# mkshing/e4t-diffusion

Hardware: NVIDIA H100
Metric: E4T pretrain images/sec @512^2 bs16 SD-v1.4 (higher is better)
Workload: dtype bf16

## Files before the change

### e4t-diffusion_b200/csrc/attention.cu

```cuda
#include "attention.cuh"
#include <math.h>
#include <stdlib.h>

static constexpr int kAttnThreads = 128;
static constexpr int kBlk = 64;

template <int DP, int NT = kAttnThreads>
__device__ __forceinline__ void load_rows(bf16* s, const bf16* g, long long ld, int rows_valid, int nrows, int dh) {
  constexpr int CPR = DP / 8, LD = DP + 8;
  const uint32_t sb = smem_u32(s);
  for (int i = threadIdx.x; i < nrows * CPR; i += NT) {
    const int r = i / CPR, c = i - r * CPR;
    const bool ok = r < rows_valid && c * 8 < dh;
    cp_async16(sb + (uint32_t)(r * LD + c * 8) * 2u, ok ? (const void*)(g + (long long)r * ld + c * 8) : (const void*)g,
               ok ? 16u : 0u);
  }
}

__device__ __forceinline__ uint32_t a_addr(const bf16* t, int LD, int row0, int col0) {
  const int l = threadIdx.x & 31;
  return smem_u32(t + (row0 + (l & 15)) * LD + col0 + (l >> 4) * 8);
}
__device__ __forceinline__ uint32_t at_addr(const bf16* t, int LD, int k0, int m0) {
  const int l = threadIdx.x & 31;
// ... 511 lines not shown
    const long long r = i / vpr;
    const int c = (int)(i % vpr) * 8;
    const float4 x = *reinterpret_cast<const float4*>(src + r * C + c);
    const float4 y = *reinterpret_cast<const float4*>(src + r * C + c + 4);
    const long long bb = r / rows_per_b, rr = r % rows_per_b;
    *reinterpret_cast<uint4*>(dst + bb * d_bs + rr * ldd + c) =
        make_uint4(pack_bf16(x.x, x.y), pack_bf16(x.z, x.w), pack_bf16(y.x, y.y), pack_bf16(y.z, y.w));
  }
}

#define E4T_ATTN_DPS(X) X(16) X(32) X(48) X(64) X(80) X(96) X(128) X(160) X(192)
static int attn_dp(int dh) {
  static const int dps[] = {16, 32, 48, 64, 80, 96, 128, 160, 192};
  for (int d : dps)
    if (dh <= d) return d;
  return 0;
}

static int env_int(const char* name, int dflt) {
  const char* e = getenv(name);
  return (e && *e) ? atoi(e) : dflt;
}

static bool attn_use_wgmma(int N, int M, int dh) {
  if (!attn_wgmma_shape_ok(N, M, dh) || !env_int("E4T_ATTN_WGMMA", 1)) return false;
  for (const char* v : {"E4T_ATTN_FWD2", "E4T_ATTN_FWD_PT", "E4T_ATTN_CG", "E4T_ATTN_BWD_FUSED", "E4T_ATTN_BWD_BQ",
                        "E4T_ATTN_BWD_STAGES"})
    if (getenv(v)) return false;
  return true;
}

static int attn_common_checks(int dh, long long ldq, long long ldk, long long ldv) {
  E4T_CHECK(dh % 8 == 0 && dh >= 8 && dh <= 192, "attention: head dim %d unsupported (need dh %% 8 == 0, <= 192)", dh);
  E4T_CHECK(ldq % 8 == 0 && ldk % 8 == 0 && ldv % 8 == 0, "attention: row strides must be multiples of 8 elements");
  return 0;
}

template <typename Kern>
static int attn_launch(Kern kernel, dim3 grid, size_t smem, const AttnArgs& a, cudaStream_t st,
                       int threads = kAttnThreads) {
  E4T_CHECK(smem <= 227 * 1024, "attention: shared memory budget exceeded (%zu)", smem);
  E4T_CUDA(cudaFuncSetAttribute(kernel, cudaFuncAttributeMaxDynamicSharedMemorySize, (int)smem));
  kernel<<<grid, threads, smem, st>>>(a);
  E4T_COUNT_LAUNCH();
  E4T_LAUNCH_CHECK();
  return 0;
}

// ... 7 lines not shown
                                                                     ldo, o_bs, lddo, do_bs);
  E4T_COUNT_LAUNCH();
}

static AttnArgs attn_args(const void* Q, const void* K, const void* V, int B, int H, int N, int M, int dh, long long ldq,
                          long long q_bs, long long ldk, long long k_bs, long long ldv, long long v_bs, float scale) {
  AttnArgs a;
  memset(&a, 0, sizeof(a));
  a.B = B; a.H = H; a.N = N; a.M = M; a.dh = dh; a.scale = scale;
  a.Q = (const bf16*)Q; a.ldq = ldq; a.q_bs = q_bs;
  a.K = (const bf16*)K; a.ldk = ldk; a.k_bs = k_bs;
  a.V = (const bf16*)V; a.ldv = ldv; a.v_bs = v_bs;
  return a;
}

extern "C" int e4t_attn_fwd(const void* Q, const void* K, const void* V, void* O, float* LSE, int B, int H, int N,
                            int M, int dh, long long ldq, long long q_bs, long long ldk, long long k_bs,
                            long long ldv, long long v_bs, long long ldo, long long o_bs, float scale,
                            void* stream_) {
  cudaStream_t st = (cudaStream_t)stream_;
  if (int e = attn_common_checks(dh, ldq, ldk, ldv)) return e;
  AttnArgs a = attn_args(Q, K, V, B, H, N, M, dh, ldq, q_bs, ldk, k_bs, ldv, v_bs, scale);
  a.O = (bf16*)O; a.ldo = ldo; a.o_bs = o_bs; a.LSE = LSE;
  if (attn_use_wgmma(N, M, dh)) return attn_wgmma_fwd(a, st);
  a.stages = 2;
  int warps = 4, cap = 0;
  if (const char* e = getenv("E4T_ATTN_FWD2")) {
    if (e[0] == '0') {
      a.stages = 1;
      warps = 8;
    } else if (e[0] == 'd' || e[0] == 's') {
      a.stages = e[0] == 's' ? 1 : 2;
      a.lazy = 1;
      for (const char* c = e + 1; *c; ++c) {
        if (*c == 'n') a.lazy = 0;
        else if (*c == 'f') warps = 8;
        else if (*c == 'p' && c[1] >= '0' && c[1] <= '8') a.poly = *++c - '0';
      }
    }
  }
  a.p_smem = env_int("E4T_ATTN_FWD_PT", 1) == 0;
  if (const char* e = getenv("E4T_ATTN_CG")) {
    int f = 4, q = 4, k = 4, o = 0;
    sscanf(e, "%d,%d,%d,%d", &f, &q, &k, &o);
    warps = f == 8 ? 8 : 4;
    cap = o > 0 ? o : 0;
  }
// ... 18 lines not shown
static int attn_bwd_impl(const void* Q, const void* K, const void* V, const void* O, const void* dO, const float* LSE,
                         float* Dv, float* dQacc, void* dQ, void* dK, void* dV, int B, int H, int N, int M, int dh,
                         long long ldq, long long q_bs, long long ldk, long long k_bs, long long ldv, long long v_bs,
                         long long ldo, long long o_bs, long long lddo, long long do_bs, long long lddq, long long dq_bs,
                         long long lddk, long long dk_bs, long long lddv, long long dv_bs, float scale, bool fused,
                         bool causal, cudaStream_t st) {
  if (int e = attn_common_checks(dh, ldq, ldk, ldv)) return e;
  E4T_CHECK(lddo % 8 == 0 && lddq % 8 == 0 && lddk % 8 == 0 && lddv % 8 == 0, "e4t_attn_bwd: strides %% 8");
  E4T_CHECK(!causal || N == M, "e4t_attn_bwd_fused_causal: needs N == M");
  AttnArgs a = attn_args(Q, K, V, B, H, N, M, dh, ldq, q_bs, ldk, k_bs, ldv, v_bs, scale);
  a.dO = (const bf16*)dO; a.lddo = lddo; a.do_bs = do_bs;
  a.LSE = const_cast<float*>(LSE); a.Dv = Dv; a.dQacc = dQacc;
  a.dQ = (bf16*)dQ; a.lddq = lddq; a.dq_bs = dq_bs;
  a.dK = (bf16*)dK; a.lddk = lddk; a.dk_bs = dk_bs;
  a.dV = (bf16*)dV; a.lddv = lddv; a.dv_bs = dv_bs;
  launch_attn_delta(O, dO, Dv, B, H, N, dh, ldo, o_bs, lddo, do_bs, st);
  E4T_LAUNCH_CHECK();
  if (fused) E4T_CUDA(cudaMemsetAsync(dQacc, 0, (size_t)B * N * H * dh * sizeof(float), st));
  a.stages = env_int("E4T_ATTN_BWD_STAGES", 2) == 1 ? 1 : 2;
  const bool bq32 = env_int("E4T_ATTN_BWD_BQ", 64) == 32;
  const dim3 gkv(cdiv(M, kBlk), H, B), gq(cdiv(N, kBlk), H, B);
  const int dp = attn_dp(dh);
  int r = -1;
  const bool wg = fused && !causal && attn_use_wgmma(N, M, dh);
  if (wg) r = attn_wgmma_bwd(a, st);
#define E4T_BWD_KV(D, BQ, S)                                                                                     \
  {                                                                                                              \
    const size_t skv = BwdCfg<D, BQ>::smem_bytes(fused);                                                         \
    if (causal) r = attn_launch(attn_bwd_kv_kernel<D, BQ, true, true, S>, gkv, skv, a, st);                      \
    else if (fused) r = attn_launch(attn_bwd_kv_kernel<D, BQ, true, false, S>, gkv, skv, a, st);                 \
    else if (!(r = attn_launch(attn_bwd_kv_kernel<D, BQ, false, false, S>, gkv, skv, a, st)))                    \
      r = attn_launch(attn_bwd_q_kernel<D>, gq, (size_t)6 * kBlk * (D + 8) * 2, a, st);                          \
  }
#define E4T_BWD_BQ(D, BQ)                                                                                        \
  {                                                                                                              \
    if (a.stages == 2) E4T_BWD_KV(D, BQ, 2)                                                                      \
    else E4T_BWD_KV(D, BQ, 1)                                                                                    \
  }
#define E4T_BWD(D)                                                                                               \
  if (!wg && dp == D) {                                                                                               \
    if (D <= 96 && !bq32) E4T_BWD_BQ(D, (D <= 96 ? 64 : 32))                                                      \
    else E4T_BWD_BQ(D, 32)                                                                                       \
  }
  E4T_ATTN_DPS(E4T_BWD)
#undef E4T_BWD
#undef E4T_BWD_BQ
#undef E4T_BWD_KV
// ... 45 lines not shown
```

### e4t-diffusion_b200/csrc/attention.cuh

```cuda
#pragma once
#include "common.cuh"

static constexpr float kLog2e = 1.4426950408889634f;

struct AttnArgs {
  int B, H, N, M, dh;
  float scale;
  int stages, lazy, poly, p_smem;
  const bf16* Q; long long ldq, q_bs;
  const bf16* K; long long ldk, k_bs;
  const bf16* V; long long ldv, v_bs;
  bf16* O; long long ldo, o_bs;
  const bf16* dO; long long lddo, do_bs;
  float* LSE;
  const float* Dv;
  float* dQacc;
  bf16* dQ; long long lddq, dq_bs;
  bf16* dK; long long lddk, dk_bs;
  bf16* dV; long long lddv, dv_bs;
};

bool attn_wgmma_shape_ok(int N, int M, int dh);
int attn_wgmma_fwd(const AttnArgs& a, cudaStream_t st);
int attn_wgmma_bwd(const AttnArgs& a, cudaStream_t st);
```

### e4t-diffusion_b200/csrc/attention_wgmma.cu

```cuda
#include "attention.cuh"
#include "wgmma.cuh"

static constexpr int kWgThreads = 384;
static constexpr int kFwdStages = 3;
static constexpr int kBwdStages = 3;
static constexpr int kTile128 = 128 * 128;
static constexpr int kTile64 = 64 * 128;

__device__ __forceinline__ uint8_t* align1024(uint8_t* p) {
  return p + ((1024u - (smem_u32(p) & 1023u)) & 1023u);
}

__device__ __forceinline__ void fwd_softmax(float (&s)[64], float (&m)[2], float (&l)[2], float (&alpha)[2], float sl2) {
#pragma unroll
  for (int hr = 0; hr < 2; ++hr) {
    float mx = -INFINITY;
#pragma unroll
    for (int j = 0; j < 16; ++j) mx = fmaxf(mx, fmaxf(s[4 * j + 2 * hr], s[4 * j + 2 * hr + 1]));
    mx = fmaxf(mx, __shfl_xor_sync(0xffffffffu, mx, 1));
    mx = fmaxf(mx, __shfl_xor_sync(0xffffffffu, mx, 2));
    const float mnew = fmaxf(m[hr], mx * sl2);
    alpha[hr] = ex2_approx(m[hr] - mnew);
    m[hr] = mnew;
    float rs = 0.f;
#pragma unroll
    for (int j = 0; j < 16; ++j)
#pragma unroll
      for (int e = 0; e < 2; ++e) {
        const float p = ex2_approx(fmaf(s[4 * j + 2 * hr + e], sl2, -mnew));
        s[4 * j + 2 * hr + e] = p;
        rs += p;
      }
    l[hr] = l[hr] * alpha[hr] + rs;
  }
}

template <int NJ>
__device__ __forceinline__ void pack_acc(const float* s, uint32_t* p) {
#pragma unroll
  for (int i = 0; i < 2 * NJ; ++i) p[i] = pack_bf16(s[2 * i], s[2 * i + 1]);
}

template <int DH>
__global__ void __launch_bounds__(kWgThreads, 1)
attn_wgmma_fwd_kernel(const __grid_constant__ CUtensorMap mapQ, const __grid_constant__ CUtensorMap mapK,
                      const __grid_constant__ CUtensorMap mapV, const AttnArgs a) {
  constexpr int KS = (DH + 15) / 16, NO = DH;
  constexpr uint32_t kStage = 2 * kTile128;
  extern __shared__ __align__(1024) uint8_t smem_raw[];
  uint8_t* smem = align1024(smem_raw);
  uint64_t* q_bar = reinterpret_cast<uint64_t*>(smem + kTile128 + kFwdStages * kStage);
  uint64_t* full_bar = q_bar + 1;
  uint64_t* empty_bar = full_bar + kFwdStages;
  const int wg = threadIdx.x >> 7;
  const int b = blockIdx.z, h = blockIdx.y, q0 = blockIdx.x * 128;
  const int nblk = a.M / 128;
  if (threadIdx.x == 0) {
    tma_prefetch_desc(&mapQ);
    tma_prefetch_desc(&mapK);
    tma_prefetch_desc(&mapV);
    mbar_init(q_bar, 1);
    for (int i = 0; i < kFwdStages; ++i) {
      mbar_init(&full_bar[i], 1);
      mbar_init(&empty_bar[i], 256);
    }
    fence_mbar_init();
  }
  __syncthreads();

  if (wg == 0) {
    setmaxnreg_dec<24>();
    if (threadIdx.x != 0) return;
    mbar_expect_tx(q_bar, kTile128);
    tma_load_4d(smem, &mapQ, q_bar, 0, h, q0, b);
    int s = 0;
    uint32_t ph = 0;
    for (int j = 0; j < nblk; ++j) {
      mbar_wait(&empty_bar[s], ph ^ 1u);
      uint8_t* sK = smem + kTile128 + s * kStage;
      mbar_expect_tx(&full_bar[s], kStage);
      tma_load_4d(sK, &mapK, &full_bar[s], 0, h, j * 128, b);
      tma_load_4d(sK + kTile128, &mapV, &full_bar[s], 0, h, j * 128, b);
      if (++s == kFwdStages) {
        s = 0;
        ph ^= 1u;
      }
    }
    return;
  }

  setmaxnreg_inc<240>();
  const int cw = wg - 1;
  const int lane = threadIdx.x & 31, warp = (threadIdx.x >> 5) & 3;
  const uint32_t s0 = smem_u32(smem);
  const uint64_t descQ = wgmma_desc(s0 + kTile64 * cw, 16, 1024);
  const uint64_t descK = wgmma_desc(s0 + kTile128, 16, 1024);
  const uint64_t descV = wgmma_desc(s0 + 2 * kTile128, kTile64, 1024);
  const float sl2 = a.scale * kLog2e;
  float s[64], o[NO / 2];
  uint32_t p[32];
  float m_r[2] = {-INFINITY, -INFINITY}, l_r[2] = {0.f, 0.f}, alpha[2];
#pragma unroll
  for (int i = 0; i < NO / 2; ++i) o[i] = 0.f;

  auto issue_qk = [&](int st) {
    const uint64_t dk = descK + (uint64_t)(st * (kStage >> 4));
#pragma unroll
    for (int k = 0; k < KS; ++k) Wgmma<128, 0, 0>::mma(s, descQ + (uint64_t)(2 * k), dk + (uint64_t)(2 * k), k > 0);
    wgmma_commit();
  };

  mbar_wait(q_bar, 0);
  mbar_wait(&full_bar[0], 0);
  wgmma_fence();
  issue_qk(0);
  wgmma_wait<0>();
  reg_fence<64>(s);
  fwd_softmax(s, m_r, l_r, alpha, sl2);
  pack_acc<16>(s, p);

  auto issue_pv = [&](int st) {
    const uint64_t dv = descV + (uint64_t)(st * (kStage >> 4));
#pragma unroll
    for (int kk = 0; kk < 8; ++kk) WgmmaRS<NO, 1>::mma(o, p + 4 * kk, dv + (uint64_t)(kk * (2048 >> 4)), 1);
    wgmma_commit();
  };
  int st = 0;
  uint32_t ph = 0;
  for (int j = 0; j + 1 < nblk; ++j) {
    int sn = st + 1;
    uint32_t phn = ph;
// ... 35 lines not shown
  reg_fence_u32<32>(p);

#pragma unroll
  for (int hr = 0; hr < 2; ++hr) {
    float l = l_r[hr];
    l += __shfl_xor_sync(0xffffffffu, l, 1);
    l += __shfl_xor_sync(0xffffffffu, l, 2);
    const int row = q0 + 64 * cw + 16 * warp + (lane >> 2) + 8 * hr;
    const float inv = 1.f / l;
    bf16* orow = a.O + b * a.o_bs + (long long)row * a.ldo + h * DH;
#pragma unroll
    for (int dt = 0; dt < DH / 8; ++dt)
      *reinterpret_cast<uint32_t*>(orow + dt * 8 + 2 * (lane & 3)) =
          pack_bf16(o[4 * dt + 2 * hr] * inv, o[4 * dt + 2 * hr + 1] * inv);
    if ((lane & 3) == 0) a.LSE[((long long)b * a.H + h) * a.N + row] = (m_r[hr] + log2f(l)) * (1.f / kLog2e);
  }
}

template <int DH>
__global__ void __launch_bounds__(kWgThreads, 1)
attn_wgmma_bwd_kernel(const __grid_constant__ CUtensorMap mapQ, const __grid_constant__ CUtensorMap mapK,
                      const __grid_constant__ CUtensorMap mapV, const __grid_constant__ CUtensorMap mapdO,
                      const __grid_constant__ CUtensorMap mapdQ, const AttnArgs a) {
  constexpr int KS = (DH + 15) / 16, NO = DH, BQ = 64;
  constexpr uint32_t kStage = 2 * kTile64;
  constexpr uint32_t kOffQ = 2 * kTile128;
  constexpr uint32_t kOffdS = kOffQ + kBwdStages * kStage;
  constexpr uint32_t kOffdQ = kOffdS + 2 * kTile128;
  constexpr uint32_t kdQBytes = BQ * DH * 4;
  constexpr uint32_t kOffL = kOffdQ + 2 * kdQBytes;
  constexpr uint32_t kOffBar = kOffL + kBwdStages * 2 * BQ * 4;
  static_assert(kOffdQ % 128 == 0 && kdQBytes % 128 == 0 && kOffL % 16 == 0 && kOffBar % 8 == 0, "smem layout");
  extern __shared__ __align__(1024) uint8_t smem_raw[];
  uint8_t* smem = align1024(smem_raw);
  float* sL = reinterpret_cast<float*>(smem + kOffL);
  uint64_t* kv_bar = reinterpret_cast<uint64_t*>(smem + kOffBar);
  uint64_t* full_bar = kv_bar + 1;
  uint64_t* empty_bar = full_bar + kBwdStages;
  uint64_t* ds_full = empty_bar + kBwdStages;
  uint64_t* ds_empty = ds_full + 2;
  const int wg = threadIdx.x >> 7;
  const int b = blockIdx.z, h = blockIdx.y, k0 = blockIdx.x * 128;
  const int lane = threadIdx.x & 31, warp = (threadIdx.x >> 5) & 3;
  const int nq = a.N / BQ;
  const long long bh = (long long)b * a.H + h;
  if (threadIdx.x == 0) {
    tma_prefetch_desc(&mapQ);
    tma_prefetch_desc(&mapK);
    tma_prefetch_desc(&mapV);
    tma_prefetch_desc(&mapdO);
    tma_prefetch_desc(&mapdQ);
    mbar_init(kv_bar, 1);
    for (int i = 0; i < kBwdStages; ++i) {
      mbar_init(&full_bar[i], 1);
      mbar_init(&empty_bar[i], 256);
    }
    for (int i = 0; i < 2; ++i) {
      mbar_init(&ds_full[i], 256);
      mbar_init(&ds_empty[i], 128);
    }
    fence_mbar_init();
  }
  __syncthreads();
  const uint32_t s0 = smem_u32(smem);

  if (wg == 0) {
    setmaxnreg_dec<72>();
    auto load_block = [&](int i) {
      const int s = i % kBwdStages;
      mbar_wait(&empty_bar[s], ((uint32_t)(i / kBwdStages) & 1u) ^ 1u);
      uint8_t* sQ = smem + kOffQ + s * kStage;
      mbar_expect_tx(&full_bar[s], kStage + 2 * BQ * 4);
      tma_load_4d(sQ, &mapQ, &full_bar[s], 0, h, i * BQ, b);
      tma_load_4d(sQ + kTile64, &mapdO, &full_bar[s], 0, h, i * BQ, b);
      bulk_load_1d(sL + s * 2 * BQ, a.LSE + bh * a.N + i * BQ, BQ * 4, &full_bar[s]);
      bulk_load_1d(sL + s * 2 * BQ + BQ, a.Dv + bh * a.N + i * BQ, BQ * 4, &full_bar[s]);
    };
    if (threadIdx.x == 0) {
      mbar_expect_tx(kv_bar, 2 * kTile128);
      tma_load_4d(smem, &mapK, kv_bar, 0, h, k0, b);
      tma_load_4d(smem + kTile128, &mapV, kv_bar, 0, h, k0, b);
      for (int i = 0; i < kBwdStages - 1 && i < nq; ++i) load_block(i);
    }
    __syncwarp();
    const uint64_t descS = wgmma_desc(s0 + kOffdS, kTile64, 1024);
    const uint64_t descK = wgmma_desc(s0, kTile64, 1024);
    mbar_wait(kv_bar, 0);
    float dq[NO / 2];
    for (int i = 0; i < nq; ++i) {
      const int buf = i & 1;
      if (threadIdx.x == 0 && i + kBwdStages - 1 < nq) load_block(i + kBwdStages - 1);
      __syncwarp();
      mbar_wait(&ds_full[buf], (uint32_t)(i >> 1) & 1u);
      const uint64_t da = descS + (uint64_t)(buf * (kTile128 >> 4));
      wgmma_fence();
#pragma unroll
      for (int kk = 0; kk < 8; ++kk)
        Wgmma<NO, 1, 1>::mma(dq, da + (uint64_t)(kk * (2048 >> 4)), descK + (uint64_t)(kk * (2048 >> 4)), kk > 0);
      wgmma_commit();
      wgmma_wait<0>();
      reg_fence<NO / 2>(dq);
      mbar_arrive(&ds_empty[buf]);
      if (threadIdx.x == 0) tma_store_wait_read<1>();
      named_bar_sync(1, 128);
      float* stg = reinterpret_cast<float*>(smem + kOffdQ + buf * kdQBytes);
#pragma unroll
      for (int hr = 0; hr < 2; ++hr) {
        float* row = stg + (16 * warp + (lane >> 2) + 8 * hr) * DH + 2 * (lane & 3);
#pragma unroll
        for (int dt = 0; dt < DH / 8; ++dt)
          *reinterpret_cast<float2*>(row + 8 * dt) =
              make_float2(dq[4 * dt + 2 * hr] * a.scale, dq[4 * dt + 2 * hr + 1] * a.scale);
      }
      fence_proxy_async_smem();
      named_bar_sync(1, 128);
      if (threadIdx.x == 0) {
        tma_reduce_add_3d(&mapdQ, stg, h * DH, i * BQ, b);
        tma_store_commit();
      }
    }
    if (threadIdx.x == 0) tma_store_wait_all();
    return;
  }

  setmaxnreg_inc<216>();
  const int cw = wg - 1;
  const uint64_t descKa = wgmma_desc(s0 + kTile64 * cw, 16, 1024);
  const uint64_t descVa = wgmma_desc(s0 + kTile128 + kTile64 * cw, 16, 1024);
  const uint64_t descQk = wgmma_desc(s0 + kOffQ, 16, 1024);
  const uint64_t descQm = wgmma_desc(s0 + kOffQ, kTile64, 1024);
  const float sl2 = a.scale * kLog2e;
  float st[32], dpt[32], dk[NO / 2], dv[NO / 2];
  uint32_t pp[16], ps[16];
#pragma unroll
  for (int i = 0; i < NO / 2; ++i) dk[i] = dv[i] = 0.f;
  const int r0 = 64 * cw + 16 * warp + (lane >> 2);
  mbar_wait(kv_bar, 0);
  for (int i = 0; i < nq; ++i) {
    const int s = i % kBwdStages, buf = i & 1;
    mbar_wait(&full_bar[s], (uint32_t)(i / kBwdStages) & 1u);
    const uint64_t so = (uint64_t)(s * (kStage >> 4));
    reg_fence<32>(st);
    reg_fence<32>(dpt);
    wgmma_fence();
#pragma unroll
    for (int k = 0; k < KS; ++k)
      Wgmma<64, 0, 0>::mma(st, descKa + (uint64_t)(2 * k), descQk + so + (uint64_t)(2 * k), k > 0);
    wgmma_commit();
#pragma unroll
    for (int k = 0; k < KS; ++k)
      Wgmma<64, 0, 0>::mma(dpt, descVa + (uint64_t)(2 * k), descQk + so + (uint64_t)((kTile64 >> 4) + 2 * k), k > 0);
    wgmma_commit();
    const float* l_s = sL + s * 2 * BQ + 2 * (lane & 3);
    wgmma_wait<1>();
    reg_fence<32>(st);
#pragma unroll
    for (int j = 0; j < 8; ++j) {
      const float2 l = *reinterpret_cast<const float2*>(l_s + 8 * j);
      const float l0 = l.x * kLog2e, l1 = l.y * kLog2e;
      st[4 * j] = ex2_approx(fmaf(st[4 * j], sl2, -l0));
      st[4 * j + 1] = ex2_approx(fmaf(st[4 * j + 1], sl2, -l1));
      st[4 * j + 2] = ex2_approx(fmaf(st[4 * j + 2], sl2, -l0));
      st[4 * j + 3] = ex2_approx(fmaf(st[4 * j + 3], sl2, -l1));
    }
    pack_acc<8>(st, pp);
    wgmma_wait<0>();
    reg_fence<32>(dpt);
#pragma unroll
    for (int j = 0; j < 8; ++j) {
      const float2 d = *reinterpret_cast<const float2*>(l_s + BQ + 8 * j);
      dpt[4 * j] = st[4 * j] * (dpt[4 * j] - d.x);
      dpt[4 * j + 1] = st[4 * j + 1] * (dpt[4 * j + 1] - d.y);
      dpt[4 * j + 2] = st[4 * j + 2] * (dpt[4 * j + 2] - d.x);
      dpt[4 * j + 3] = st[4 * j + 3] * (dpt[4 * j + 3] - d.y);
    }
    pack_acc<8>(dpt, ps);
    mbar_wait(&ds_empty[buf], ((uint32_t)(i >> 1) & 1u) ^ 1u);
    uint8_t* sdS = smem + kOffdS + buf * kTile128;
#pragma unroll
    for (int j = 0; j < 8; ++j) {
      *reinterpret_cast<uint32_t*>(sdS + sw128_off(r0, j) + 4 * (lane & 3)) = ps[2 * j];
      *reinterpret_cast<uint32_t*>(sdS + sw128_off(r0 + 8, j) + 4 * (lane & 3)) = ps[2 * j + 1];
    }
    fence_proxy_async_smem();
    mbar_arrive(&ds_full[buf]);
    reg_fence<NO / 2>(dk);
    reg_fence<NO / 2>(dv);
    wgmma_fence();
#pragma unroll
    for (int kq = 0; kq < 4; ++kq)
      WgmmaRS<NO, 1>::mma(dv, pp + 4 * kq, descQm + so + (uint64_t)((kTile64 >> 4) + kq * (2048 >> 4)), 1);
#pragma unroll
    for (int kq = 0; kq < 4; ++kq) WgmmaRS<NO, 1>::mma(dk, ps + 4 * kq, descQm + so + (uint64_t)(kq * (2048 >> 4)), 1);
    wgmma_commit();
    wgmma_wait<0>();
    reg_fence<NO / 2>(dk);
    reg_fence<NO / 2>(dv);
    reg_fence_u32<16>(pp);
    reg_fence_u32<16>(ps);
    mbar_arrive(&empty_bar[s]);
  }
#pragma unroll
  for (int hr = 0; hr < 2; ++hr) {
    const int key = k0 + r0 + 8 * hr;
    bf16* dkr = a.dK + b * a.dk_bs + (long long)key * a.lddk + h * DH + 2 * (lane & 3);
    bf16* dvr = a.dV + b * a.dv_bs + (long long)key * a.lddv + h * DH + 2 * (lane & 3);
#pragma unroll
    for (int dt = 0; dt < DH / 8; ++dt) {
      *reinterpret_cast<uint32_t*>(dkr + 8 * dt) = pack_bf16(dk[4 * dt + 2 * hr] * a.scale, dk[4 * dt + 2 * hr + 1] * a.scale);
      *reinterpret_cast<uint32_t*>(dvr + 8 * dt) = pack_bf16(dv[4 * dt + 2 * hr], dv[4 * dt + 2 * hr + 1]);
    }
  }
}

bool attn_wgmma_shape_ok(int N, int M, int dh) {
  return dh == 40 && N >= 512 && M >= 512 && N % 128 == 0 && M % 128 == 0;
}

static int head_map(CUtensorMap* m, const bf16* p, const AttnArgs& a, int tokens, long long ld, long long bs, int rows) {
  E4T_CHECK(((uintptr_t)p & 15) == 0 && ld % 8 == 0 && bs % 8 == 0,
            "attention (wgmma): tensors must be 16-byte aligned with strides that are multiples of 8 elements");
  const uint64_t dims[4] = {(uint64_t)a.dh, (uint64_t)a.H, (uint64_t)tokens, (uint64_t)a.B};
  const uint64_t str[3] = {(uint64_t)a.dh * 2, (uint64_t)ld * 2, (uint64_t)bs * 2};
  const uint32_t box[4] = {64, 1, (uint32_t)rows, 1};
  return e4t_tmap_encode(m, p, 4, dims, str, box, 2);
}

int attn_wgmma_fwd(const AttnArgs& a, cudaStream_t st) {
  CUtensorMap mQ, mK, mV;
  if (int e = head_map(&mQ, a.Q, a, a.N, a.ldq, a.q_bs, 128)) return e;
  if (int e = head_map(&mK, a.K, a, a.M, a.ldk, a.k_bs, 128)) return e;
  if (int e = head_map(&mV, a.V, a, a.M, a.ldv, a.v_bs, 128)) return e;
  E4T_CHECK(a.ldo % 2 == 0 && a.o_bs % 2 == 0, "attention (wgmma): output strides must be even");
  const size_t smem = 1024 + kTile128 + kFwdStages * 2 * kTile128 + 64;
  auto kernel = attn_wgmma_fwd_kernel<40>;
  E4T_CUDA(cudaFuncSetAttribute(kernel, cudaFuncAttributeMaxDynamicSharedMemorySize, (int)smem));
  kernel<<<dim3(a.N / 128, a.H, a.B), kWgThreads, smem, st>>>(mQ, mK, mV, a);
  E4T_COUNT_LAUNCH();
  E4T_LAUNCH_CHECK();
  return 0;
}

int attn_wgmma_bwd(const AttnArgs& a, cudaStream_t st) {
  CUtensorMap mQ, mK, mV, mdO, mdQ;
  if (int e = head_map(&mQ, a.Q, a, a.N, a.ldq, a.q_bs, 64)) return e;
  if (int e = head_map(&mK, a.K, a, a.M, a.ldk, a.k_bs, 128)) return e;
  if (int e = head_map(&mV, a.V, a, a.M, a.ldv, a.v_bs, 128)) return e;
  if (int e = head_map(&mdO, a.dO, a, a.N, a.lddo, a.do_bs, 64)) return e;
  {
    const uint64_t C = (uint64_t)a.H * a.dh;
    const uint64_t dims[3] = {C, (uint64_t)a.N, (uint64_t)a.B};
    const uint64_t str[2] = {C * 4, (uint64_t)a.N * C * 4};
    const uint32_t box[3] = {(uint32_t)a.dh, 64, 1};
    E4T_CHECK(((uintptr_t)a.dQacc & 15) == 0 && ((uintptr_t)a.LSE & 15) == 0 && ((uintptr_t)a.Dv & 15) == 0,
              "attention (wgmma): LSE, D and dQ scratch must be 16-byte aligned");
    if (int e = e4t_tmap_encode(&mdQ, a.dQacc, 3, dims, str, box, 4, 0)) return e;
  }
  E4T_CHECK(a.lddk % 2 == 0 && a.dk_bs % 2 == 0 && a.lddv % 2 == 0 && a.dv_bs % 2 == 0,
            "attention (wgmma): gradient strides must be even");
  const size_t smem = 1024 + 2 * kTile128 + kBwdStages * 2 * kTile64 + 2 * kTile128 + 2 * 64 * 40 * 4 +
                      kBwdStages * 2 * 64 * 4 + 128;
  auto kernel = attn_wgmma_bwd_kernel<40>;
  E4T_CUDA(cudaFuncSetAttribute(kernel, cudaFuncAttributeMaxDynamicSharedMemorySize, (int)smem));
  kernel<<<dim3(a.M / 128, a.H, a.B), kWgThreads, smem, st>>>(mQ, mK, mV, mdO, mdQ, a);
  E4T_COUNT_LAUNCH();
  E4T_LAUNCH_CHECK();
  return 0;
}
```

### e4t-diffusion_b200/csrc/wgmma.cuh

```cuda
#pragma once
#include <stdint.h>

template <int N, int TA, int TB>
struct Wgmma;

template <int TA, int TB>
struct Wgmma<64, TA, TB> {
  static __device__ __forceinline__ void mma(float* d, uint64_t da, uint64_t db, uint32_t scale_d) {
    asm volatile(
        "{\n\t.reg .pred p;\n\tsetp.ne.b32 p, %34, 0;\n\t"
        "wgmma.mma_async.sync.aligned.m64n64k16.f32.bf16.bf16 {%0, %1, %2, %3, %4, %5, %6, %7, %8, %9, %10, %11, %12, %13, %14, %15, %16, %17, %18, %19, %20, %21, %22, %23, %24, %25, %26, %27, %28, %29, %30, %31}, %32, %33, p, 1, 1, %35, %36;\n\t}"
        : "+f"(d[0]), "+f"(d[1]), "+f"(d[2]), "+f"(d[3]), "+f"(d[4]), "+f"(d[5]), "+f"(d[6]), "+f"(d[7]), "+f"(d[8]), "+f"(d[9]), "+f"(d[10]), "+f"(d[11]), "+f"(d[12]), "+f"(d[13]), "+f"(d[14]), "+f"(d[15]), "+f"(d[16]), "+f"(d[17]), "+f"(d[18]), "+f"(d[19]), "+f"(d[20]), "+f"(d[21]), "+f"(d[22]), "+f"(d[23]), "+f"(d[24]), "+f"(d[25]), "+f"(d[26]), "+f"(d[27]), "+f"(d[28]), "+f"(d[29]), "+f"(d[30]), "+f"(d[31])
        : "l"(da), "l"(db), "r"(scale_d), "n"(TA), "n"(TB));
  }
};

template <int TA, int TB>
struct Wgmma<96, TA, TB> {
  static __device__ __forceinline__ void mma(float* d, uint64_t da, uint64_t db, uint32_t scale_d) {
    asm volatile(
        "{\n\t.reg .pred p;\n\tsetp.ne.b32 p, %50, 0;\n\t"
        "wgmma.mma_async.sync.aligned.m64n96k16.f32.bf16.bf16 {%0, %1, %2, %3, %4, %5, %6, %7, %8, %9, %10, %11, %12, %13, %14, %15, %16, %17, %18, %19, %20, %21, %22, %23, %24, %25, %26, %27, %28, %29, %30, %31, %32, %33, %34, %35, %36, %37, %38, %39, %40, %41, %42, %43, %44, %45, %46, %47}, %48, %49, p, 1, 1, %51, %52;\n\t}"
        : "+f"(d[0]), "+f"(d[1]), "+f"(d[2]), "+f"(d[3]), "+f"(d[4]), "+f"(d[5]), "+f"(d[6]), "+f"(d[7]), "+f"(d[8]), "+f"(d[9]), "+f"(d[10]), "+f"(d[11]), "+f"(d[12]), "+f"(d[13]), "+f"(d[14]), "+f"(d[15]), "+f"(d[16]), "+f"(d[17]), "+f"(d[18]), "+f"(d[19]), "+f"(d[20]), "+f"(d[21]), "+f"(d[22]), "+f"(d[23]), "+f"(d[24]), "+f"(d[25]), "+f"(d[26]), "+f"(d[27]), "+f"(d[28]), "+f"(d[29]), "+f"(d[30]), "+f"(d[31]), "+f"(d[32]), "+f"(d[33]), "+f"(d[34]), "+f"(d[35]), "+f"(d[36]), "+f"(d[37]), "+f"(d[38]), "+f"(d[39]), "+f"(d[40]), "+f"(d[41]), "+f"(d[42]), "+f"(d[43]), "+f"(d[44]), "+f"(d[45]), "+f"(d[46]), "+f"(d[47])
        : "l"(da), "l"(db), "r"(scale_d), "n"(TA), "n"(TB));
// ... 46 lines not shown

template <int TA, int TB>
struct Wgmma<256, TA, TB> {
  static __device__ __forceinline__ void mma(float* d, uint64_t da, uint64_t db, uint32_t scale_d) {
    asm volatile(
        "{\n\t.reg .pred p;\n\tsetp.ne.b32 p, %130, 0;\n\t"
        "wgmma.mma_async.sync.aligned.m64n256k16.f32.bf16.bf16 {%0, %1, %2, %3, %4, %5, %6, %7, %8, %9, %10, %11, %12, %13, %14, %15, %16, %17, %18, %19, %20, %21, %22, %23, %24, %25, %26, %27, %28, %29, %30, %31, %32, %33, %34, %35, %36, %37, %38, %39, %40, %41, %42, %43, %44, %45, %46, %47, %48, %49, %50, %51, %52, %53, %54, %55, %56, %57, %58, %59, %60, %61, %62, %63, %64, %65, %66, %67, %68, %69, %70, %71, %72, %73, %74, %75, %76, %77, %78, %79, %80, %81, %82, %83, %84, %85, %86, %87, %88, %89, %90, %91, %92, %93, %94, %95, %96, %97, %98, %99, %100, %101, %102, %103, %104, %105, %106, %107, %108, %109, %110, %111, %112, %113, %114, %115, %116, %117, %118, %119, %120, %121, %122, %123, %124, %125, %126, %127}, %128, %129, p, 1, 1, %131, %132;\n\t}"
        : "+f"(d[0]), "+f"(d[1]), "+f"(d[2]), "+f"(d[3]), "+f"(d[4]), "+f"(d[5]), "+f"(d[6]), "+f"(d[7]), "+f"(d[8]), "+f"(d[9]), "+f"(d[10]), "+f"(d[11]), "+f"(d[12]), "+f"(d[13]), "+f"(d[14]), "+f"(d[15]), "+f"(d[16]), "+f"(d[17]), "+f"(d[18]), "+f"(d[19]), "+f"(d[20]), "+f"(d[21]), "+f"(d[22]), "+f"(d[23]), "+f"(d[24]), "+f"(d[25]), "+f"(d[26]), "+f"(d[27]), "+f"(d[28]), "+f"(d[29]), "+f"(d[30]), "+f"(d[31]), "+f"(d[32]), "+f"(d[33]), "+f"(d[34]), "+f"(d[35]), "+f"(d[36]), "+f"(d[37]), "+f"(d[38]), "+f"(d[39]), "+f"(d[40]), "+f"(d[41]), "+f"(d[42]), "+f"(d[43]), "+f"(d[44]), "+f"(d[45]), "+f"(d[46]), "+f"(d[47]), "+f"(d[48]), "+f"(d[49]), "+f"(d[50]), "+f"(d[51]), "+f"(d[52]), "+f"(d[53]), "+f"(d[54]), "+f"(d[55]), "+f"(d[56]), "+f"(d[57]), "+f"(d[58]), "+f"(d[59]), "+f"(d[60]), "+f"(d[61]), "+f"(d[62]), "+f"(d[63]), "+f"(d[64]), "+f"(d[65]), "+f"(d[66]), "+f"(d[67]), "+f"(d[68]), "+f"(d[69]), "+f"(d[70]), "+f"(d[71]), "+f"(d[72]), "+f"(d[73]), "+f"(d[74]), "+f"(d[75]), "+f"(d[76]), "+f"(d[77]), "+f"(d[78]), "+f"(d[79]), "+f"(d[80]), "+f"(d[81]), "+f"(d[82]), "+f"(d[83]), "+f"(d[84]), "+f"(d[85]), "+f"(d[86]), "+f"(d[87]), "+f"(d[88]), "+f"(d[89]), "+f"(d[90]), "+f"(d[91]), "+f"(d[92]), "+f"(d[93]), "+f"(d[94]), "+f"(d[95]), "+f"(d[96]), "+f"(d[97]), "+f"(d[98]), "+f"(d[99]), "+f"(d[100]), "+f"(d[101]), "+f"(d[102]), "+f"(d[103]), "+f"(d[104]), "+f"(d[105]), "+f"(d[106]), "+f"(d[107]), "+f"(d[108]), "+f"(d[109]), "+f"(d[110]), "+f"(d[111]), "+f"(d[112]), "+f"(d[113]), "+f"(d[114]), "+f"(d[115]), "+f"(d[116]), "+f"(d[117]), "+f"(d[118]), "+f"(d[119]), "+f"(d[120]), "+f"(d[121]), "+f"(d[122]), "+f"(d[123]), "+f"(d[124]), "+f"(d[125]), "+f"(d[126]), "+f"(d[127])
        : "l"(da), "l"(db), "r"(scale_d), "n"(TA), "n"(TB));
  }
};

template <int TA, int TB>
struct Wgmma<40, TA, TB> {
  static __device__ __forceinline__ void mma(float* d, uint64_t da, uint64_t db, uint32_t scale_d) {
    asm volatile(
        "{\n\t.reg .pred p;\n\tsetp.ne.b32 p, %22, 0;\n\t"
        "wgmma.mma_async.sync.aligned.m64n40k16.f32.bf16.bf16 {%0, %1, %2, %3, %4, %5, %6, %7, %8, %9, %10, %11, %12, %13, %14, %15, %16, %17, %18, %19}, %20, %21, p, 1, 1, %23, %24;\n\t}"
        : "+f"(d[0]), "+f"(d[1]), "+f"(d[2]), "+f"(d[3]), "+f"(d[4]), "+f"(d[5]), "+f"(d[6]), "+f"(d[7]), "+f"(d[8]), "+f"(d[9]), "+f"(d[10]), "+f"(d[11]), "+f"(d[12]), "+f"(d[13]), "+f"(d[14]), "+f"(d[15]), "+f"(d[16]), "+f"(d[17]), "+f"(d[18]), "+f"(d[19])
        : "l"(da), "l"(db), "r"(scale_d), "n"(TA), "n"(TB));
  }
};

template <int N, int TB>
struct WgmmaRS;

template <int TB>
struct WgmmaRS<40, TB> {
  static __device__ __forceinline__ void mma(float* d, const uint32_t* a, uint64_t db, uint32_t scale_d) {
    asm volatile(
        "{\n\t.reg .pred p;\n\tsetp.ne.b32 p, %25, 0;\n\t"
        "wgmma.mma_async.sync.aligned.m64n40k16.f32.bf16.bf16 {%0, %1, %2, %3, %4, %5, %6, %7, %8, %9, %10, %11, %12, %13, %14, %15, %16, %17, %18, %19}, {%20, %21, %22, %23}, %24, p, 1, 1, %26;\n\t}"
        : "+f"(d[0]), "+f"(d[1]), "+f"(d[2]), "+f"(d[3]), "+f"(d[4]), "+f"(d[5]), "+f"(d[6]), "+f"(d[7]), "+f"(d[8]), "+f"(d[9]), "+f"(d[10]), "+f"(d[11]), "+f"(d[12]), "+f"(d[13]), "+f"(d[14]), "+f"(d[15]), "+f"(d[16]), "+f"(d[17]), "+f"(d[18]), "+f"(d[19])
        : "r"(a[0]), "r"(a[1]), "r"(a[2]), "r"(a[3]), "l"(db), "r"(scale_d), "n"(TB));
  }
};
```

Before: 104.9.

## Extend WGMMA/TMA warp-specialized attention to head dim 80

After: 108.4 (median of 6 runs). +3.3%, better.

```diff
diff --git a/e4t-diffusion_b200/csrc/attention.cu b/e4t-diffusion_b200/csrc/attention.cu
--- a/e4t-diffusion_b200/csrc/attention.cu
+++ b/e4t-diffusion_b200/csrc/attention.cu
@@ -557,8 +557,8 @@
   return (e && *e) ? atoi(e) : dflt;
 }
 
-static bool attn_use_wgmma(int N, int M, int dh) {
-  if (!attn_wgmma_shape_ok(N, M, dh) || !env_int("E4T_ATTN_WGMMA", 1)) return false;
+static bool attn_use_wgmma(int B, int H, int N, int M, int dh) {
+  if (!attn_wgmma_shape_ok(B, H, N, M, dh) || !env_int("E4T_ATTN_WGMMA", 1)) return false;
   for (const char* v : {"E4T_ATTN_FWD2", "E4T_ATTN_FWD_PT", "E4T_ATTN_CG", "E4T_ATTN_BWD_FUSED", "E4T_ATTN_BWD_BQ",
                         "E4T_ATTN_BWD_STAGES"})
     if (getenv(v)) return false;
@@ -612,7 +612,7 @@
   if (int e = attn_common_checks(dh, ldq, ldk, ldv)) return e;
   AttnArgs a = attn_args(Q, K, V, B, H, N, M, dh, ldq, q_bs, ldk, k_bs, ldv, v_bs, scale);
   a.O = (bf16*)O; a.ldo = ldo; a.o_bs = o_bs; a.LSE = LSE;
-  if (attn_use_wgmma(N, M, dh)) return attn_wgmma_fwd(a, st);
+  if (attn_use_wgmma(B, H, N, M, dh)) return attn_wgmma_fwd(a, st);
   a.stages = 2;
   int warps = 4, cap = 0;
   if (const char* e = getenv("E4T_ATTN_FWD2")) {
@@ -677,7 +677,7 @@
   const dim3 gkv(cdiv(M, kBlk), H, B), gq(cdiv(N, kBlk), H, B);
   const int dp = attn_dp(dh);
   int r = -1;
-  const bool wg = fused && !causal && attn_use_wgmma(N, M, dh);
+  const bool wg = fused && !causal && attn_use_wgmma(B, H, N, M, dh);
   if (wg) r = attn_wgmma_bwd(a, st);
 #define E4T_BWD_KV(D, BQ, S)                                                                                     \
   {                                                                                                              \
diff --git a/e4t-diffusion_b200/csrc/attention.cuh b/e4t-diffusion_b200/csrc/attention.cuh
--- a/e4t-diffusion_b200/csrc/attention.cuh
+++ b/e4t-diffusion_b200/csrc/attention.cuh
@@ -20,6 +20,6 @@
   bf16* dV; long long lddv, dv_bs;
 };
 
-bool attn_wgmma_shape_ok(int N, int M, int dh);
+bool attn_wgmma_shape_ok(int B, int H, int N, int M, int dh);
 int attn_wgmma_fwd(const AttnArgs& a, cudaStream_t st);
 int attn_wgmma_bwd(const AttnArgs& a, cudaStream_t st);
diff --git a/e4t-diffusion_b200/csrc/attention_wgmma.cu b/e4t-diffusion_b200/csrc/attention_wgmma.cu
--- a/e4t-diffusion_b200/csrc/attention_wgmma.cu
+++ b/e4t-diffusion_b200/csrc/attention_wgmma.cu
@@ -3,13 +3,47 @@
 
 static constexpr int kWgThreads = 384;
 static constexpr int kFwdStages = 3;
-static constexpr int kBwdStages = 3;
 static constexpr int kTile128 = 128 * 128;
 static constexpr int kTile64 = 64 * 128;
+static constexpr size_t kMaxSmem = 227 * 1024;
+
+__device__ __forceinline__ constexpr uint64_t kstep(int k, uint32_t panel) {
+  return (uint64_t)((k / 4) * (panel >> 4) + 2 * (k % 4));
+}
 
 __device__ __forceinline__ uint8_t* align1024(uint8_t* p) {
   return p + ((1024u - (smem_u32(p) & 1023u)) & 1023u);
 }
+
+template <int DH>
+struct FwdSmem {
+  static constexpr int P = (DH + 63) / 64;
+  static constexpr uint32_t kTile = P * kTile128;
+  static constexpr uint32_t kStage = 2 * kTile;
+  static constexpr uint32_t kOffBar = kTile + kFwdStages * kStage;
+  static constexpr size_t bytes = 1024 + kOffBar + 8 * (1 + 2 * kFwdStages);
+  static constexpr uint32_t kLboV = P > 1 ? kTile128 : kTile64;
+  static_assert(bytes <= kMaxSmem, "forward shared memory");
+};
+
+template <int DH>
+struct BwdSmem {
+  static constexpr int P = (DH + 63) / 64, BQ = 64;
+  static constexpr int kStages = P > 1 ? 2 : 3;
+  static constexpr uint32_t kKV = P * kTile128;
+  static constexpr uint32_t kQ = P * kTile64;
+  static constexpr uint32_t kStage = 2 * kQ;
+  static constexpr uint32_t kOffQ = 2 * kKV;
+  static constexpr uint32_t kOffdS = kOffQ + kStages * kStage;
+  static constexpr uint32_t kOffdQ = kOffdS + 2 * kTile128;
+  static constexpr uint32_t kdQBytes = BQ * DH * 4;
+  static constexpr uint32_t kOffL = kOffdQ + 2 * kdQBytes;
+  static constexpr uint32_t kOffBar = kOffL + kStages * 2 * BQ * 4;
+  static constexpr size_t bytes = 1024 + kOffBar + 8 * (1 + 2 * kStages + 4);
+  static constexpr uint32_t kLboK = P > 1 ? kTile128 : kTile64;
+  static_assert(kOffdQ % 128 == 0 && kdQBytes % 128 == 0 && kOffL % 16 == 0 && kOffBar % 8 == 0, "smem layout");
+  static_assert(bytes <= kMaxSmem, "backward shared memory");
+};
 
 __device__ __forceinline__ void fwd_softmax(float (&s)[64], float (&m)[2], float (&l)[2], float (&alpha)[2], float sl2) {
 #pragma unroll
@@ -45,11 +79,12 @@
 __global__ void __launch_bounds__(kWgThreads, 1)
 attn_wgmma_fwd_kernel(const __grid_constant__ CUtensorMap mapQ, const __grid_constant__ CUtensorMap mapK,
                       const __grid_constant__ CUtensorMap mapV, const AttnArgs a) {
+  using L = FwdSmem<DH>;
   constexpr int KS = (DH + 15) / 16, NO = DH;
-  constexpr uint32_t kStage = 2 * kTile128;
+  constexpr uint32_t kStage = L::kStage;
   extern __shared__ __align__(1024) uint8_t smem_raw[];
   uint8_t* smem = align1024(smem_raw);
-  uint64_t* q_bar = reinterpret_cast<uint64_t*>(smem + kTile128 + kFwdStages * kStage);
+  uint64_t* q_bar = reinterpret_cast<uint64_t*>(smem + L::kOffBar);
   uint64_t* full_bar = q_bar + 1;
   uint64_t* empty_bar = full_bar + kFwdStages;
   const int wg = threadIdx.x >> 7;
@@ -71,16 +106,20 @@
   if (wg == 0) {
     setmaxnreg_dec<24>();
     if (threadIdx.x != 0) return;
-    mbar_expect_tx(q_bar, kTile128);
-    tma_load_4d(smem, &mapQ, q_bar, 0, h, q0, b);
+    mbar_expect_tx(q_bar, L::kTile);
+#pragma unroll
+    for (int pn = 0; pn < L::P; ++pn) tma_load_4d(smem + pn * kTile128, &mapQ, q_bar, 64 * pn, h, q0, b);
     int s = 0;
     uint32_t ph = 0;
     for (int j = 0; j < nblk; ++j) {
       mbar_wait(&empty_bar[s], ph ^ 1u);
-      uint8_t* sK = smem + kTile128 + s * kStage;
+      uint8_t* sK = smem + L::kTile + s * kStage;
       mbar_expect_tx(&full_bar[s], kStage);
-      tma_load_4d(sK, &mapK, &full_bar[s], 0, h, j * 128, b);
-      tma_load_4d(sK + kTile128, &mapV, &full_bar[s], 0, h, j * 128, b);
+#pragma unroll
+      for (int pn = 0; pn < L::P; ++pn) {
+        tma_load_4d(sK + pn * kTile128, &mapK, &full_bar[s], 64 * pn, h, j * 128, b);
+        tma_load_4d(sK + L::kTile + pn * kTile128, &mapV, &full_bar[s], 64 * pn, h, j * 128, b);
+      }
       if (++s == kFwdStages) {
         s = 0;
         ph ^= 1u;
@@ -94,8 +133,8 @@
   const int lane = threadIdx.x & 31, warp = (threadIdx.x >> 5) & 3;
   const uint32_t s0 = smem_u32(smem);
   const uint64_t descQ = wgmma_desc(s0 + kTile64 * cw, 16, 1024);
-  const uint64_t descK = wgmma_desc(s0 + kTile128, 16, 1024);
-  const uint64_t descV = wgmma_desc(s0 + 2 * kTile128, kTile64, 1024);
+  const uint64_t descK = wgmma_desc(s0 + L::kTile, 16, 1024);
+  const uint64_t descV = wgmma_desc(s0 + 2 * L::kTile, L::kLboV, 1024);
   const float sl2 = a.scale * kLog2e;
   float s[64], o[NO / 2];
   uint32_t p[32];
@@ -106,7 +145,7 @@
   auto issue_qk = [&](int st) {
     const uint64_t dk = descK + (uint64_t)(st * (kStage >> 4));
 #pragma unroll
-    for (int k = 0; k < KS; ++k) Wgmma<128, 0, 0>::mma(s, descQ + (uint64_t)(2 * k), dk + (uint64_t)(2 * k), k > 0);
+    for (int k = 0; k < KS; ++k) Wgmma<128, 0, 0>::mma(s, descQ + kstep(k, kTile128), dk + kstep(k, kTile128), k > 0);
     wgmma_commit();
   };
 
@@ -188,15 +227,10 @@
 attn_wgmma_bwd_kernel(const __grid_constant__ CUtensorMap mapQ, const __grid_constant__ CUtensorMap mapK,
                       const __grid_constant__ CUtensorMap mapV, const __grid_constant__ CUtensorMap mapdO,
                       const __grid_constant__ CUtensorMap mapdQ, const AttnArgs a) {
-  constexpr int KS = (DH + 15) / 16, NO = DH, BQ = 64;
-  constexpr uint32_t kStage = 2 * kTile64;
-  constexpr uint32_t kOffQ = 2 * kTile128;
-  constexpr uint32_t kOffdS = kOffQ + kBwdStages * kStage;
-  constexpr uint32_t kOffdQ = kOffdS + 2 * kTile128;
-  constexpr uint32_t kdQBytes = BQ * DH * 4;
-  constexpr uint32_t kOffL = kOffdQ + 2 * kdQBytes;
-  constexpr uint32_t kOffBar = kOffL + kBwdStages * 2 * BQ * 4;
-  static_assert(kOffdQ % 128 == 0 && kdQBytes % 128 == 0 && kOffL % 16 == 0 && kOffBar % 8 == 0, "smem layout");
+  using L = BwdSmem<DH>;
+  constexpr int KS = (DH + 15) / 16, NO = DH, BQ = L::BQ, kBwdStages = L::kStages;
+  constexpr uint32_t kStage = L::kStage, kOffQ = L::kOffQ, kOffdS = L::kOffdS, kOffdQ = L::kOffdQ;
+  constexpr uint32_t kdQBytes = L::kdQBytes, kOffL = L::kOffL, kOffBar = L::kOffBar;
   extern __shared__ __align__(1024) uint8_t smem_raw[];
   uint8_t* smem = align1024(smem_raw);
   float* sL = reinterpret_cast<float*>(smem + kOffL);
@@ -237,20 +271,26 @@
       mbar_wait(&empty_bar[s], ((uint32_t)(i / kBwdStages) & 1u) ^ 1u);
       uint8_t* sQ = smem + kOffQ + s * kStage;
       mbar_expect_tx(&full_bar[s], kStage + 2 * BQ * 4);
-      tma_load_4d(sQ, &mapQ, &full_bar[s], 0, h, i * BQ, b);
-      tma_load_4d(sQ + kTile64, &mapdO, &full_bar[s], 0, h, i * BQ, b);
+#pragma unroll
+      for (int pn = 0; pn < L::P; ++pn) {
+        tma_load_4d(sQ + pn * kTile64, &mapQ, &full_bar[s], 64 * pn, h, i * BQ, b);
+        tma_load_4d(sQ + L::kQ + pn * kTile64, &mapdO, &full_bar[s], 64 * pn, h, i * BQ, b);
+      }
       bulk_load_1d(sL + s * 2 * BQ, a.LSE + bh * a.N + i * BQ, BQ * 4, &full_bar[s]);
       bulk_load_1d(sL + s * 2 * BQ + BQ, a.Dv + bh * a.N + i * BQ, BQ * 4, &full_bar[s]);
     };
     if (threadIdx.x == 0) {
-      mbar_expect_tx(kv_bar, 2 * kTile128);
-      tma_load_4d(smem, &mapK, kv_bar, 0, h, k0, b);
-      tma_load_4d(smem + kTile128, &mapV, kv_bar, 0, h, k0, b);
+      mbar_expect_tx(kv_bar, 2 * L::kKV);
+#pragma unroll
+      for (int pn = 0; pn < L::P; ++pn) {
+        tma_load_4d(smem + pn * kTile128, &mapK, kv_bar, 64 * pn, h, k0, b);
+        tma_load_4d(smem + L::kKV + pn * kTile128, &mapV, kv_bar, 64 * pn, h, k0, b);
+      }
       for (int i = 0; i < kBwdStages - 1 && i < nq; ++i) load_block(i);
     }
     __syncwarp();
     const uint64_t descS = wgmma_desc(s0 + kOffdS, kTile64, 1024);
-    const uint64_t descK = wgmma_desc(s0, kTile64, 1024);
+    const uint64_t descK = wgmma_desc(s0, L::kLboK, 1024);
     mbar_wait(kv_bar, 0);
     float dq[NO / 2];
     for (int i = 0; i < nq; ++i) {
@@ -292,7 +332,7 @@
   setmaxnreg_inc<216>();
   const int cw = wg - 1;
   const uint64_t descKa = wgmma_desc(s0 + kTile64 * cw, 16, 1024);
-  const uint64_t descVa = wgmma_desc(s0 + kTile128 + kTile64 * cw, 16, 1024);
+  const uint64_t descVa = wgmma_desc(s0 + L::kKV + kTile64 * cw, 16, 1024);
   const uint64_t descQk = wgmma_desc(s0 + kOffQ, 16, 1024);
   const uint64_t descQm = wgmma_desc(s0 + kOffQ, kTile64, 1024);
   const float sl2 = a.scale * kLog2e;
@@ -311,11 +351,11 @@
     wgmma_fence();
 #pragma unroll
     for (int k = 0; k < KS; ++k)
-      Wgmma<64, 0, 0>::mma(st, descKa + (uint64_t)(2 * k), descQk + so + (uint64_t)(2 * k), k > 0);
+      Wgmma<64, 0, 0>::mma(st, descKa + kstep(k, kTile128), descQk + so + kstep(k, kTile64), k > 0);
     wgmma_commit();
 #pragma unroll
     for (int k = 0; k < KS; ++k)
-      Wgmma<64, 0, 0>::mma(dpt, descVa + (uint64_t)(2 * k), descQk + so + (uint64_t)((kTile64 >> 4) + 2 * k), k > 0);
+      Wgmma<64, 0, 0>::mma(dpt, descVa + kstep(k, kTile128), descQk + so + (L::kQ >> 4) + kstep(k, kTile64), k > 0);
     wgmma_commit();
     const float* l_s = sL + s * 2 * BQ + 2 * (lane & 3);
     wgmma_wait<1>();
@@ -355,7 +395,7 @@
     wgmma_fence();
 #pragma unroll
     for (int kq = 0; kq < 4; ++kq)
-      WgmmaRS<NO, 1>::mma(dv, pp + 4 * kq, descQm + so + (uint64_t)((kTile64 >> 4) + kq * (2048 >> 4)), 1);
+      WgmmaRS<NO, 1>::mma(dv, pp + 4 * kq, descQm + so + (uint64_t)((L::kQ >> 4) + kq * (2048 >> 4)), 1);
 #pragma unroll
     for (int kq = 0; kq < 4; ++kq) WgmmaRS<NO, 1>::mma(dk, ps + 4 * kq, descQm + so + (uint64_t)(kq * (2048 >> 4)), 1);
     wgmma_commit();
@@ -379,8 +419,14 @@
   }
 }
 
-bool attn_wgmma_shape_ok(int N, int M, int dh) {
-  return dh == 40 && N >= 512 && M >= 512 && N % 128 == 0 && M % 128 == 0;
+bool attn_wgmma_shape_ok(int B, int H, int N, int M, int dh) {
+  if (!(dh == 40 || dh == 80) || N < 512 || M < 512 || N % 128 != 0 || M % 128 != 0) return false;
+  if (dh == 40) return true;
+  int sms = 0, dev = 0;
+  cudaGetDevice(&dev);
+  cudaDeviceGetAttribute(&sms, cudaDevAttrMultiProcessorCount, dev);
+  if (sms <= 0) sms = 132;
+  return 2LL * (N / 128) * H * B >= sms;
 }
 
 static int head_map(CUtensorMap* m, const bf16* p, const AttnArgs& a, int tokens, long long ld, long long bs, int rows) {
@@ -398,8 +444,8 @@
   if (int e = head_map(&mK, a.K, a, a.M, a.ldk, a.k_bs, 128)) return e;
   if (int e = head_map(&mV, a.V, a, a.M, a.ldv, a.v_bs, 128)) return e;
   E4T_CHECK(a.ldo % 2 == 0 && a.o_bs % 2 == 0, "attention (wgmma): output strides must be even");
-  const size_t smem = 1024 + kTile128 + kFwdStages * 2 * kTile128 + 64;
-  auto kernel = attn_wgmma_fwd_kernel<40>;
+  const size_t smem = a.dh == 40 ? FwdSmem<40>::bytes : FwdSmem<80>::bytes;
+  auto kernel = a.dh == 40 ? attn_wgmma_fwd_kernel<40> : attn_wgmma_fwd_kernel<80>;
   E4T_CUDA(cudaFuncSetAttribute(kernel, cudaFuncAttributeMaxDynamicSharedMemorySize, (int)smem));
   kernel<<<dim3(a.N / 128, a.H, a.B), kWgThreads, smem, st>>>(mQ, mK, mV, a);
   E4T_COUNT_LAUNCH();
@@ -424,9 +470,8 @@
   }
   E4T_CHECK(a.lddk % 2 == 0 && a.dk_bs % 2 == 0 && a.lddv % 2 == 0 && a.dv_bs % 2 == 0,
             "attention (wgmma): gradient strides must be even");
-  const size_t smem = 1024 + 2 * kTile128 + kBwdStages * 2 * kTile64 + 2 * kTile128 + 2 * 64 * 40 * 4 +
-                      kBwdStages * 2 * 64 * 4 + 128;
-  auto kernel = attn_wgmma_bwd_kernel<40>;
+  const size_t smem = a.dh == 40 ? BwdSmem<40>::bytes : BwdSmem<80>::bytes;
+  auto kernel = a.dh == 40 ? attn_wgmma_bwd_kernel<40> : attn_wgmma_bwd_kernel<80>;
   E4T_CUDA(cudaFuncSetAttribute(kernel, cudaFuncAttributeMaxDynamicSharedMemorySize, (int)smem));
   kernel<<<dim3(a.M / 128, a.H, a.B), kWgThreads, smem, st>>>(mQ, mK, mV, mdO, mdQ, a);
   E4T_COUNT_LAUNCH();
diff --git a/e4t-diffusion_b200/csrc/wgmma.cuh b/e4t-diffusion_b200/csrc/wgmma.cuh
--- a/e4t-diffusion_b200/csrc/wgmma.cuh
+++ b/e4t-diffusion_b200/csrc/wgmma.cuh
@@ -92,6 +92,17 @@
   }
 };
 
+template <int TA, int TB>
+struct Wgmma<80, TA, TB> {
+  static __device__ __forceinline__ void mma(float* d, uint64_t da, uint64_t db, uint32_t scale_d) {
+    asm volatile(
+        "{\n\t.reg .pred p;\n\tsetp.ne.b32 p, %42, 0;\n\t"
+        "wgmma.mma_async.sync.aligned.m64n80k16.f32.bf16.bf16 {%0, %1, %2, %3, %4, %5, %6, %7, %8, %9, %10, %11, %12, %13, %14, %15, %16, %17, %18, %19, %20, %21, %22, %23, %24, %25, %26, %27, %28, %29, %30, %31, %32, %33, %34, %35, %36, %37, %38, %39}, %40, %41, p, 1, 1, %43, %44;\n\t}"
+        : "+f"(d[0]), "+f"(d[1]), "+f"(d[2]), "+f"(d[3]), "+f"(d[4]), "+f"(d[5]), "+f"(d[6]), "+f"(d[7]), "+f"(d[8]), "+f"(d[9]), "+f"(d[10]), "+f"(d[11]), "+f"(d[12]), "+f"(d[13]), "+f"(d[14]), "+f"(d[15]), "+f"(d[16]), "+f"(d[17]), "+f"(d[18]), "+f"(d[19]), "+f"(d[20]), "+f"(d[21]), "+f"(d[22]), "+f"(d[23]), "+f"(d[24]), "+f"(d[25]), "+f"(d[26]), "+f"(d[27]), "+f"(d[28]), "+f"(d[29]), "+f"(d[30]), "+f"(d[31]), "+f"(d[32]), "+f"(d[33]), "+f"(d[34]), "+f"(d[35]), "+f"(d[36]), "+f"(d[37]), "+f"(d[38]), "+f"(d[39])
+        : "l"(da), "l"(db), "r"(scale_d), "n"(TA), "n"(TB));
+  }
+};
+
 template <int N, int TB>
 struct WgmmaRS;
 
@@ -105,3 +116,14 @@
         : "r"(a[0]), "r"(a[1]), "r"(a[2]), "r"(a[3]), "l"(db), "r"(scale_d), "n"(TB));
   }
 };
+
+template <int TB>
+struct WgmmaRS<80, TB> {
+  static __device__ __forceinline__ void mma(float* d, const uint32_t* a, uint64_t db, uint32_t scale_d) {
+    asm volatile(
+        "{\n\t.reg .pred p;\n\tsetp.ne.b32 p, %45, 0;\n\t"
+        "wgmma.mma_async.sync.aligned.m64n80k16.f32.bf16.bf16 {%0, %1, %2, %3, %4, %5, %6, %7, %8, %9, %10, %11, %12, %13, %14, %15, %16, %17, %18, %19, %20, %21, %22, %23, %24, %25, %26, %27, %28, %29, %30, %31, %32, %33, %34, %35, %36, %37, %38, %39}, {%40, %41, %42, %43}, %44, p, 1, 1, %46;\n\t}"
+        : "+f"(d[0]), "+f"(d[1]), "+f"(d[2]), "+f"(d[3]), "+f"(d[4]), "+f"(d[5]), "+f"(d[6]), "+f"(d[7]), "+f"(d[8]), "+f"(d[9]), "+f"(d[10]), "+f"(d[11]), "+f"(d[12]), "+f"(d[13]), "+f"(d[14]), "+f"(d[15]), "+f"(d[16]), "+f"(d[17]), "+f"(d[18]), "+f"(d[19]), "+f"(d[20]), "+f"(d[21]), "+f"(d[22]), "+f"(d[23]), "+f"(d[24]), "+f"(d[25]), "+f"(d[26]), "+f"(d[27]), "+f"(d[28]), "+f"(d[29]), "+f"(d[30]), "+f"(d[31]), "+f"(d[32]), "+f"(d[33]), "+f"(d[34]), "+f"(d[35]), "+f"(d[36]), "+f"(d[37]), "+f"(d[38]), "+f"(d[39])
+        : "r"(a[0]), "r"(a[1]), "r"(a[2]), "r"(a[3]), "l"(db), "r"(scale_d), "n"(TB));
+  }
+};
```
